# cyberfabric/cyberfabric-core

Measured on AMD Instinct MI355X. Metric: tokens/sec + p50 TTFT via llm-gateway REST /v1/chat/completions, higher is better.
Workload: dtype bf16; 1 GPU; model=llama3-8b, global_batch=2048, seq_len=512, parallelism=dp1(worker fleet)

## Files before the change

csrc/bindings.cpp:

```cpp
#include <torch/extension.h>

#include <c10/hip/HIPStream.h>
#include <hip/hip_bf16.h>

#include <stdexcept>

using bf16 = __hip_bfloat16;

void launch_rmsnorm(bf16*, const bf16*, const bf16*, float, long, int,
                    hipStream_t);
void launch_fused_add_rmsnorm(bf16*, bf16*, const bf16*, float, long, int,
                              hipStream_t);
void launch_rope_kv_append(bf16*, bf16*, const bf16*, const long*,
                           const float*, const long*, bf16*, bf16*, long,
                           int, int, int, int, long, long, long, bool,
                           hipStream_t);
void launch_paged_attn(bf16*, const bf16*, const bf16*, const bf16*,
                       const int*, const int*, const int*, long, int, int,
                       int, int, int, float, long, float*, int, bool,
                       hipStream_t);
void launch_attn_prefill_mfma(bf16*, const bf16*, const bf16*,
                              const bf16*, const int*, int, int, int, int,
                              int, float, long, long, long, hipStream_t);
void launch_attn_prefill_paged_mfma(bf16*, const bf16*, const bf16*,
                                    const bf16*, const int*, const int*,
                                    const int*, int, int, int, int, int, int,
                                    int, float, long, bool, hipStream_t);
void launch_silu_mul(bf16*, const bf16*, long, int, hipStream_t);
void launch_quant_fp8(unsigned char*, float*, const bf16*, long, int, long,
                      hipStream_t);
void launch_fused_add_rmsnorm_fp8(unsigned char*, float*, const bf16*,
                                  bf16*, const bf16*, float, long, int,
                                  hipStream_t);
void launch_silu_mul_fp8(unsigned char*, float*, const bf16*, long, int,
                         hipStream_t);
void launch_moe_align(int*, int*, int*, const int*, int, int, int,
                      hipStream_t);
void launch_moe_gemm(bf16*, float*, const bf16*, const bf16*, const int*,
                     const int*, int, int, int, int, int, hipStream_t);
void launch_moe_combine(bf16*, const bf16*, const float*, const int*, long,
                        int, int, hipStream_t);
void launch_moe_gemm_fp8(bf16*, float*, const unsigned char*, const float*,
                         const unsigned char*, const float*, const int*,
                         const int*, int, int, int, int, int, hipStream_t);
void launch_greedy_sample(long*, const bf16*, long, int, hipStream_t);
void launch_inv_cdf_sample(long*, const float*, const float*, long, int,
                           hipStream_t);

namespace {

hipStream_t stream() {
  return c10::hip::getCurrentHIPStream().stream();
}

void check(const torch::Tensor& t, torch::ScalarType dt, const char* name) {
  TORCH_CHECK(t.is_cuda(), name, " must be on GPU");
  TORCH_CHECK(t.is_contiguous(), name, " must be contiguous");
  TORCH_CHECK(t.scalar_type() == dt, name, " has wrong dtype");
}

bf16* bf(torch::Tensor& t) { return reinterpret_cast<bf16*>(t.data_ptr()); }
const bf16* cbf(const torch::Tensor& t) {
  return reinterpret_cast<const bf16*>(t.data_ptr());
}

void rmsnorm(torch::Tensor out, torch::Tensor x, torch::Tensor w,
             double eps) {
  check(out, torch::kBFloat16, "out");
  check(x, torch::kBFloat16, "x");
  check(w, torch::kBFloat16, "w");
  const int hidden = (int)x.size(-1);
  TORCH_CHECK(hidden % 8 == 0 && hidden <= 16384, "hidden size");
  launch_rmsnorm(bf(out), cbf(x), cbf(w), (float)eps, x.numel() / hidden,
                 hidden, stream());
}

void fused_add_rmsnorm(torch::Tensor x, torch::Tensor residual,
                       torch::Tensor w, double eps) {
  check(x, torch::kBFloat16, "x");
  check(residual, torch::kBFloat16, "residual");
// ... 132 lines not shown
  launch_attn_prefill_paged_mfma(
      bf(out), cbf(q), cbf(k_cache), cbf(v_cache),
      block_tables.data_ptr<int>(), seq_start.data_ptr<int>(),
      ctx_start.data_ptr<int>(), S, (int)max_seqlen, H, KV,
      (int)q.size(2), (int)block_tables.size(1), (int)k_cache.size(2),
      (float)scale, q.stride(0), kv_fp8, stream());
}

void silu_mul(torch::Tensor out, torch::Tensor x) {
  check(out, torch::kBFloat16, "out");
  check(x, torch::kBFloat16, "x");
  const int inter = (int)out.size(-1);
  TORCH_CHECK(x.size(-1) == 2 * inter && inter % 8 == 0, "shape");
  launch_silu_mul(bf(out), cbf(x), out.numel() / inter, inter, stream());
}

void greedy_sample(torch::Tensor out, torch::Tensor logits) {
  check(out, torch::kInt64, "out");
  check(logits, torch::kBFloat16, "logits");
  launch_greedy_sample(out.data_ptr<long>(), cbf(logits), logits.size(0),
                       (int)logits.size(1), stream());
}

void inv_cdf_sample(torch::Tensor out, torch::Tensor logits,
                    torch::Tensor uniform) {
  check(out, torch::kInt64, "out");
  check(logits, torch::kFloat32, "logits");
  check(uniform, torch::kFloat32, "uniform");
  launch_inv_cdf_sample(out.data_ptr<long>(), logits.data_ptr<float>(),
                        uniform.data_ptr<float>(), logits.size(0),
                        (int)logits.size(1), stream());
}

}


unsigned char* u8(torch::Tensor& t) {
  return reinterpret_cast<unsigned char*>(t.data_ptr());
}

void quant_fp8(torch::Tensor out, torch::Tensor scales, torch::Tensor x) {
  check(out, torch::kFloat8_e4m3fn, "out");
  check(scales, torch::kFloat, "scales");
  TORCH_CHECK(x.is_cuda() && x.scalar_type() == torch::kBFloat16, "x");
  const int hidden = (int)x.size(-1);
  TORCH_CHECK(x.stride(-1) == 1, "x inner dim must be contiguous");
  const long rows = x.numel() / hidden;
  const long stride = x.dim() > 1 ? x.stride(0) : hidden;
  launch_quant_fp8(u8(out), scales.data_ptr<float>(), cbf(x), rows, hidden,
                   stride, stream());
}

void fused_add_rmsnorm_fp8(torch::Tensor out, torch::Tensor scales,
                           torch::Tensor x, torch::Tensor residual,
                           torch::Tensor w, double eps) {
  check(out, torch::kFloat8_e4m3fn, "out");
  check(scales, torch::kFloat, "scales");
  check(x, torch::kBFloat16, "x");
  check(residual, torch::kBFloat16, "residual");
  check(w, torch::kBFloat16, "w");
  const int hidden = (int)x.size(-1);
  launch_fused_add_rmsnorm_fp8(u8(out), scales.data_ptr<float>(), cbf(x),
                               bf(residual), cbf(w), (float)eps,
                               x.numel() / hidden, hidden, stream());
}

// ... 76 lines not shown
    TORCH_CHECK(skw.has_value(),
                "moe_gemm_fp8: splitk>1 needs a workspace");
    check(*skw, torch::kFloat, "skw");
    TORCH_CHECK(skw->numel() >= splitk * out.numel(),
                "moe_gemm_fp8: workspace too small");
    skp = skw->data_ptr<float>();
  }
  launch_moe_gemm_fp8(bf(out), skp, u8(xq), xs.data_ptr<float>(), u8(wq),
                      ws.data_ptr<float>(), sorted_ids.data_ptr<int>(),
                      tile_expert.data_ptr<int>(),
                      (int)tile_expert.numel(), (int)wq.size(1),
                      (int)wq.size(2), (int)gather_div, (int)splitk,
                      stream());
}

PYBIND11_MODULE(TORCH_EXTENSION_NAME, m) {
  m.doc() = "HyperSpot-AMD gfx950 (CDNA4) kernels";
  m.def("rmsnorm", &rmsnorm);
  m.def("quant_fp8", &quant_fp8);
  m.def("fused_add_rmsnorm_fp8", &fused_add_rmsnorm_fp8);
  m.def("silu_mul_fp8", &silu_mul_fp8);
  m.def("moe_align", &moe_align);
  m.def("moe_gemm", &moe_gemm);
  m.def("moe_combine", &moe_combine);
  m.def("moe_gemm_fp8", &moe_gemm_fp8);
  m.def("fused_add_rmsnorm", &fused_add_rmsnorm);
  m.def("rope_kv_append", &rope_kv_append);
  m.def("paged_attn", &paged_attn);
  m.def("attn_prefill_mfma", &attn_prefill_mfma);
  m.def("attn_prefill_paged_mfma", &attn_prefill_paged_mfma);
  m.def("silu_mul", &silu_mul);
  m.def("greedy_sample", &greedy_sample);
  m.def("inv_cdf_sample", &inv_cdf_sample);
}
```

hyperspot/engine/config.py:

```python

from __future__ import annotations

from dataclasses import dataclass, field
from typing import Optional


@dataclass
class ModelSpec:

    name: str
    hidden_size: int
    num_layers: int
    num_heads: int
    num_kv_heads: int
    head_dim: int
    intermediate_size: int
    vocab_size: int
    rope_theta: float = 500000.0
    rms_eps: float = 1e-5
    max_position: int = 8192
    tie_embeddings: bool = False
    num_experts: int = 0
    num_experts_per_tok: int = 0
    dtype: str = "bfloat16"
# ... 46 lines not shown
        name="tiny-moe", hidden_size=256, num_layers=2, num_heads=4,
        num_kv_heads=2, head_dim=64, intermediate_size=256, vocab_size=512,
        rope_theta=10000.0, max_position=1024, num_experts=4,
        num_experts_per_tok=2,
    ),
}


def get_model_spec(name: str) -> ModelSpec:
    key = name.lower()
    if key not in _PRESETS:
        raise KeyError(f"unknown model preset '{name}' (have: {sorted(_PRESETS)})")
    return _PRESETS[key]


@dataclass
class EngineConfig:

    model: str = "llama3-8b"
    block_size: int = 16
    max_num_seqs: int = 256
    max_num_batched_tokens: int = 8192
    max_model_len: int = 8192
    gpu_memory_utilization: float = 0.90
    num_gpu_blocks: Optional[int] = None
    enforce_eager: bool = False
    tp_size: int = 1
    ep_size: int = 1
    dtype: str = "bfloat16"
    quant: Optional[str] = None
    kv_dtype: str = "bfloat16"
    enable_prefix_caching: bool = False
    prefill_paged_mfma: bool = False
    seed: int = 0
    graph_batch_sizes: tuple = (1, 2, 4, 8, 16, 24, 32, 48, 64, 96, 128,
                                192, 256, 384, 512, 768, 1024, 1536, 2048)
    prefill_graph_sizes: tuple = (128, 256, 512, 1024, 2048)

    def spec(self) -> ModelSpec:
        return get_model_spec(self.model)


@dataclass
class SamplingParams:

    temperature: float = 1.0
    top_p: float = 1.0
    top_k: int = 0
    max_tokens: int = 128
    min_tokens: int = 0
    stop_token_ids: tuple = ()
    ignore_eos: bool = False
    seed: Optional[int] = None
    response_format: Optional[str] = None
    response_schema: Optional[dict] = None
    tool_names: tuple = ()

    @property
    def greedy(self) -> bool:
        return self.temperature == 0.0
```

hyperspot/engine/engine.py:

```python

from __future__ import annotations

import itertools
import logging
import time
from typing import List, Optional

from .config import EngineConfig, SamplingParams
from .model_runner import ModelRunner
from .request import FinishReason, Request, StepOutput
from .scheduler import Scheduler

log = logging.getLogger(__name__)


class LLMEngine:
    def __init__(self, config: EngineConfig, device: Optional[str] = None,
                 eos_token_id: Optional[int] = None):
        t0 = time.monotonic()
        self.config = config
        self.runner = ModelRunner(config, device=device)
        self.scheduler = Scheduler(config, self.runner.block_manager)
        self.eos_token_id = eos_token_id
        self._id_counter = itertools.count()
        log.info("engine up: model=%s blocks=%d device=%s (%.1fs)",
                 config.model, self.runner.num_blocks, self.runner.device,
                 time.monotonic() - t0)

    def add_request(self, prompt_token_ids: List[int],
                    sampling: Optional[SamplingParams] = None,
                    request_id: Optional[str] = None,
                    tenant_id: str = "default") -> str:
        rid = request_id or f"req-{next(self._id_counter)}"
        req = Request(request_id=rid,
                      prompt_token_ids=list(prompt_token_ids),
                      sampling=sampling or SamplingParams(),
                      tenant_id=tenant_id)
        self.scheduler.add(req)
        return rid

    def abort_request(self, request_id: str) -> None:
        self.scheduler.abort(request_id)

    def has_work(self) -> bool:
        return self.scheduler.has_work()

    @property
    def num_running(self) -> int:
        return len(self.scheduler.running)

    @property
    def num_waiting(self) -> int:
        return len(self.scheduler.waiting)

    def step(self) -> List[StepOutput]:
        batch = self.scheduler.schedule()
        if batch.empty:
            return []
        tokens = self.runner.execute(batch)
        outputs: List[StepOutput] = []
        bm = self.runner.block_manager
        for req, tok in zip(batch.requests, tokens.tolist()):
            if batch.mode == "prefill" and bm.enable_prefix_caching:
                bm.commit_hashes(req.request_id, req.num_computed_tokens)
            if batch.mode == "prefill" and \
                    req.num_computed_tokens < req.num_prompt_tokens:
                continue
            req.append_output(int(tok), self.eos_token_id)
            outputs.append(StepOutput(req.request_id, int(tok), req.finished,
                                      req.finish_reason))
        self.scheduler.finish_step()
        return outputs

    def capture_graphs(self) -> None:
        self.runner.capture_all_graphs()

    def embed(self, prompts):
        return self.runner.embed(prompts)

    def swap_weights(self, checkpoint_path: str) -> float:
        return self.runner.swap_weights(checkpoint_path)

    def save_checkpoint(self, path: str) -> None:
        from .checkpoint import save_checkpoint
        save_checkpoint(self.runner.model, path,
                        {"model": self.config.model})

    def generate(self, prompts: List[List[int]],
                 sampling: Optional[SamplingParams] = None):
        ids = [self.add_request(p, sampling) for p in prompts]
        results = {i: [] for i in ids}
        while self.has_work():
            for out in self.step():
                if out.request_id in results:
                    results[out.request_id].append(out.token_id)
        return [results[i] for i in ids]
```

hyperspot/engine/model_runner.py:

```python

from __future__ import annotations

import logging
from typing import Dict, List, Optional

import torch

from hyperspot import ops
from hyperspot.models import build_model
from hyperspot.models.llama import ForwardMeta

from .config import EngineConfig
from .kv_cache import (BlockManager, allocate_kv_caches,
                       compute_num_gpu_blocks)
from .request import Request
from .scheduler import ScheduledBatch

log = logging.getLogger(__name__)

_TUNABLEOP_LOADED = False


def _load_tunableop_results() -> None:
    global _TUNABLEOP_LOADED
    if _TUNABLEOP_LOADED:
        return
    _TUNABLEOP_LOADED = True
    import os
    path = os.path.join(os.path.dirname(os.path.dirname(
        os.path.dirname(os.path.abspath(__file__)))),
        "profiles", "tunableop_gfx950.csv")
    if not os.path.exists(path):
        return
    try:
        t = torch.cuda.tunable
        t.enable(True)
        t.tuning_enable(False)
        t.record_untuned_enable(False)
        t.read_file(path)
        log.info("TunableOp: loaded %s", path)
    except Exception as e:
        log.warning("TunableOp load failed: %s", e)


class ModelRunner:
    def __init__(self, config: EngineConfig, device: Optional[str] = None):
        self.config = config
        self.spec = config.spec()
        if config.max_model_len > self.spec.max_position:
            log.warning("max_model_len %d clamped to the model's "
                        "max_position %d", config.max_model_len,
                        self.spec.max_position)
            config.max_model_len = self.spec.max_position
        self.device = torch.device(
            device if device is not None
            else ("cuda" if torch.cuda.is_available() else "cpu"))
        self.dtype = torch.bfloat16 if self.device.type == "cuda" \
            else torch.float32
        torch.manual_seed(config.seed)
        if self.device.type == "cuda":
            _load_tunableop_results()
        from hyperspot.parallel.layers import set_init_device, set_quant_mode
        set_init_device(self.device)
        set_quant_mode(config.quant)
        self.model = build_model(self.spec, dtype=self.dtype).to(self.device)
        self.model.eval()
        self.num_blocks = compute_num_gpu_blocks(self.spec, config, self.device)
        kv_heads_local = self.spec.num_kv_heads // max(config.tp_size, 1)
        assert config.kv_dtype in ("bfloat16", "fp8"), config.kv_dtype
        kv_dt = torch.float8_e4m3fn if config.kv_dtype == "fp8"             else self.dtype
        self.kv_caches = allocate_kv_caches(
            self.spec.num_layers, self.num_blocks, kv_heads_local,
            config.block_size, self.spec.head_dim, kv_dt, self.device)
        self.max_blocks_per_seq = (config.max_model_len + config.block_size - 1) \
            // config.block_size
        self.block_manager = BlockManager(
            self.num_blocks, config.block_size,
            capacity=max(config.max_num_seqs * 2, 64),
            max_blocks_per_seq=self.max_blocks_per_seq,
            enable_prefix_caching=config.enable_prefix_caching)
        self._gen = torch.Generator().manual_seed(config.seed)
        pin = self.device.type == "cuda"
        cap = self.block_manager.capacity
        self._st_ids = torch.empty(cap, dtype=torch.long, pin_memory=pin)
        self._st_pos = torch.empty(cap, dtype=torch.long, pin_memory=pin)
        self._st_slots = torch.empty(cap, dtype=torch.long, pin_memory=pin)
        self._st_lens = torch.empty(cap, dtype=torch.int32, pin_memory=pin)
        self._st_bt_flat = torch.empty(cap * self.max_blocks_per_seq,
                                       dtype=torch.int32, pin_memory=pin)
        self._guided_mask_cache: Dict[tuple, torch.Tensor] = {}
        self._graphs: Dict[int, torch.cuda.CUDAGraph] = {}
        self._graph_io: Dict[int, dict] = {}
        self._pgraphs: Dict[int, torch.cuda.CUDAGraph] = {}
        self._pgraph_io: Dict[int, dict] = {}
        self._graph_pool = None


    def _prefill_inputs(self, batch: ScheduledBatch):
        ids: List[int] = []
        pos: List[int] = []
        slots: List[int] = []
        starts = [0]
        logit_rows = []
        import numpy as np
        row_seq: List[int] = []
        tables = []
        bm = self.block_manager
        bs = bm.block_size
        fresh = True
        ctx_start: List[int] = []
        for si, req in enumerate(batch.requests):
            cs = req.chunk_start
            n = req.chunk_len or req.num_prompt_tokens
            ctx_start.append(cs)
            if cs > 0:
                fresh = False
            ids.extend(req.prompt_token_ids[cs:cs + n])
            pos.extend(range(cs, cs + n))
            row = bm.row_of[req.request_id]
            p = np.arange(cs, cs + n)
            s = bm.tables_np[row, p // bs].astype(np.int64) * bs + p % bs
            slots.extend(s.tolist())
            starts.append(starts[-1] + n)
            logit_rows.append(starts[-1] - 1)
            row_seq.extend([si] * n)
            tables.append(bm.table(req.request_id))
        max_t = max(len(t) for t in tables)
        bt = torch.zeros(len(tables), max_t, dtype=torch.int32)
# ... 108 lines not shown
            "input_ids": torch.zeros(T, dtype=torch.long, device=d),
            "positions": torch.zeros(T, dtype=torch.long, device=d),
            "slot_mapping": torch.full((T,), -1, dtype=torch.long,
                                       device=d),
            "lidx": torch.zeros(1, dtype=torch.long, device=d),
        }
        meta = ForwardMeta(
            mode="prefill", positions=io["positions"],
            slot_mapping=io["slot_mapping"],
            seq_start=torch.tensor([0, T], dtype=torch.int32, device=d),
            max_seqlen=T, fresh_prefill=True,
            logits_indices=io["lidx"])
        for _ in range(2):
            self.model(io["input_ids"], meta, self.kv_caches)
        torch.cuda.synchronize()
        g = torch.cuda.CUDAGraph()
        with torch.cuda.graph(g, pool=self._graph_pool):
            io["logits"] = self.model(io["input_ids"], meta,
                                      self.kv_caches)
        if self._graph_pool is None:
            self._graph_pool = g.pool()
        self._pgraphs[T] = g
        self._pgraph_io[T] = io

    def _decode_forward(self, input_ids, meta):
        B = input_ids.shape[0]
        bucket = self._bucket_for(B)
        if bucket is None or self.device.type != "cuda" \
                or self.config.enforce_eager:
            return self.model(input_ids, meta, self.kv_caches)
        if bucket not in self._graphs:
            self._capture(bucket)
        io = self._graph_io[bucket]
        io["input_ids"][:B] = input_ids
        io["input_ids"][B:] = 0
        io["positions"][:B] = meta.positions
        io["positions"][B:] = 0
        io["slot_mapping"][:B] = meta.slot_mapping
        io["slot_mapping"][B:] = -1
        io["block_tables"].zero_()
        io["block_tables"][:B, :meta.block_tables.shape[1]] = meta.block_tables
        io["seq_lens"][:B] = meta.seq_lens
        io["seq_lens"][B:] = 1
        self._graphs[bucket].replay()
        return io["logits"][:B]

    def _bucket_for(self, b: int) -> Optional[int]:
        for s in self.config.graph_batch_sizes:
            if s >= b:
                return s
        return None

    def _capture(self, bucket: int) -> None:
        d = self.device
        log.info("capturing decode hipGraph for batch=%d", bucket)
        io = {
            "input_ids": torch.zeros(bucket, dtype=torch.long, device=d),
            "positions": torch.zeros(bucket, dtype=torch.long, device=d),
            "slot_mapping": torch.full((bucket,), -1, dtype=torch.long, device=d),
            "block_tables": torch.zeros(bucket, self.max_blocks_per_seq,
                                        dtype=torch.int32, device=d),
            "seq_lens": torch.ones(bucket, dtype=torch.int32, device=d),
        }
        meta = ForwardMeta(mode="decode", positions=io["positions"],
                           slot_mapping=io["slot_mapping"],
                           block_tables=io["block_tables"],
                           seq_lens=io["seq_lens"])
        for _ in range(2):
            self.model(io["input_ids"], meta, self.kv_caches)
        torch.cuda.synchronize()
        g = torch.cuda.CUDAGraph()
        with torch.cuda.graph(g, pool=self._graph_pool):
            io["logits"] = self.model(io["input_ids"], meta, self.kv_caches)
        if self._graph_pool is None:
            self._graph_pool = g.pool()
        self._graphs[bucket] = g
        self._graph_io[bucket] = io

    @torch.inference_mode()
    def capture_all_graphs(self) -> None:
        if self.device.type != "cuda" or self.config.enforce_eager:
            return
        for b in self.config.graph_batch_sizes:
            if b <= self.config.max_num_seqs and b not in self._graphs:
                self._capture(b)
        for t in self.config.prefill_graph_sizes:
            if (t <= self.config.max_num_batched_tokens
                    and t <= self.config.max_model_len
                    and t not in self._pgraphs):
                self._capture_prefill(t)


    @torch.inference_mode()
    def embed(self, prompts: List[List[int]]) -> torch.Tensor:
        from .request import Request
        from .config import SamplingParams
        bm = self.block_manager
        fake = []
        try:
            for i, p in enumerate(prompts):
                rid = f"__embed_{i}"
                bm.allocate(rid, len(p))
                fake.append(Request(request_id=rid, prompt_token_ids=list(p),
                                    sampling=SamplingParams()))
            batch = ScheduledBatch(mode="prefill", requests=fake,
                                   num_tokens=sum(len(p) for p in prompts))
            input_ids, meta = self._prefill_inputs(batch)
            meta.return_hidden = True
            hidden = self.model(input_ids, meta, self.kv_caches).float()
            out = torch.empty(len(prompts), hidden.shape[-1],
                              dtype=torch.float32, device=hidden.device)
            ss = meta.seq_start
            for i in range(len(prompts)):
                out[i] = hidden[int(ss[i]):int(ss[i + 1])].mean(0)
        finally:
            for i in range(len(prompts)):
                bm.free(f"__embed_{i}")
        return out.cpu()

    def swap_weights(self, checkpoint_path: str) -> float:
        from .checkpoint import load_checkpoint_into
        return load_checkpoint_into(self.model, checkpoint_path)

# ... 77 lines not shown
```

hyperspot/engine/scheduler.py:

```python

from __future__ import annotations

from collections import deque
from dataclasses import dataclass, field
from typing import Deque, List, Optional

from .config import EngineConfig
from .kv_cache import BlockManager
from .request import Request, RequestState


@dataclass
class ScheduledBatch:
    mode: str
    requests: List[Request] = field(default_factory=list)
    num_tokens: int = 0

    @property
    def empty(self) -> bool:
        return not self.requests


class Scheduler:
    def __init__(self, config: EngineConfig, block_manager: BlockManager):
        self.config = config
        self.bm = block_manager
        self.waiting: Deque[Request] = deque()
        self.running: List[Request] = []
        self.watermark = max(1, int(0.01 * block_manager.num_blocks))

    def add(self, req: Request) -> None:
        self.waiting.append(req)

    def abort(self, request_id: str) -> None:
        for q in (self.waiting, self.running):
            for r in list(q):
                if r.request_id == request_id:
                    q.remove(r)
                    if r.request_id in self.bm.row_of:
                        self.bm.free(r.request_id)
                    r.state = RequestState.FINISHED

    def has_work(self) -> bool:
        return bool(self.waiting or self.running)

    def schedule(self) -> ScheduledBatch:
        batch = self._schedule_prefill()
        if not batch.empty:
            return batch
        return self._schedule_decode()

    def _schedule_prefill(self) -> ScheduledBatch:
        batch = ScheduledBatch(mode="prefill")
        budget = self.config.max_num_batched_tokens
        completed = []
        while self.waiting and budget > 0:
            req = self.waiting[0]
            total = req.num_prompt_tokens
            if total > self.config.max_model_len:
                self.waiting.popleft()
                req.state = RequestState.FINISHED
                continue
            done = req.num_computed_tokens
            if done == 0 and len(self.running) + len(batch.requests)                     >= self.config.max_num_seqs:
                break
            if done == 0 and self.bm.enable_prefix_caching:
                if not self.bm.can_allocate(total, self.watermark):
                    break
                cached = self.bm.allocate_with_prefix(
                    req.request_id, total, req.prompt_token_ids)
                req.num_computed_tokens = done = cached
                req.blocks_preallocated = True
            chunk = min(total - done, budget)
            if chunk <= 0:
                break
            if getattr(req, "blocks_preallocated", False):
                pass
            elif done == 0:
                if not self.bm.can_allocate(chunk, self.watermark):
                    break
                self.bm.allocate(req.request_id, chunk)
            else:
                if not self.bm.can_extend(req.request_id, chunk,
                                          self.watermark):
                    break
                self.bm.extend(req.request_id, chunk)
            req.chunk_start, req.chunk_len = done, chunk
            req.num_computed_tokens = done + chunk
            batch.requests.append(req)
            budget -= chunk
            batch.num_tokens += chunk
            if req.num_computed_tokens == total:
                self.waiting.popleft()
                req.state = RequestState.RUNNING
                completed.append(req)
        self.running.extend(completed)
        return batch

    def _schedule_decode(self) -> ScheduledBatch:
        batch = ScheduledBatch(mode="decode")
        while self.running:
            need = sum(1 for req in self.running
                       if self.bm.tokens_of(req.request_id)
                       % self.bm.block_size == 0)
            if need <= self.bm.num_free:
                break
            victim = self.running.pop()
            self.bm.free(victim.request_id)
            victim.state = RequestState.PREEMPTED
            victim.prompt_token_ids = victim.prompt_token_ids + victim.output_token_ids
            victim.output_token_ids = []
            victim.num_computed_tokens = 0
            victim.blocks_preallocated = False
            self.waiting.appendleft(victim)
        batch.requests = list(self.running)
        batch.num_tokens = len(batch.requests)
        return batch

    def finish_step(self) -> List[Request]:
        done = [r for r in self.running if r.finished]
        for r in done:
            self.bm.free(r.request_id)
        self.running = [r for r in self.running if not r.finished]
        return done
```

hyperspot/ops/__init__.py:

```python

from __future__ import annotations

from typing import NamedTuple

import torch

from . import torch_ref

_C = None
_C_ERR: Exception | None = None
try:
    from hyperspot import _C as _C
except Exception as e:
    _C_ERR = e


def have_native() -> bool:
    return _C is not None


def _native():
    if _C is None:
        raise RuntimeError(
            "hyperspot._C (gfx950 HIP extension) is not built but a GPU tensor "
# ... 197 lines not shown

def moe_ffn_fp8(xq: "QTensor", w13q: torch.Tensor, w13s: torch.Tensor,
                w2q: torch.Tensor, w2s: torch.Tensor,
                weights: torch.Tensor, ids: torch.Tensor) -> torch.Tensor:
    T, H = xq.data.shape
    K = ids.shape[1]
    E = w13q.shape[0]
    TK = T * K
    ntiles = (TK + E * (MOE_BM - 1) + MOE_BM - 1) // MOE_BM
    P = ntiles * MOE_BM
    dev = xq.data.device
    flat = ids.reshape(-1).to(torch.int32)
    sorted_ids = torch.empty(P, dtype=torch.int32, device=dev)
    tile_expert = torch.empty(ntiles, dtype=torch.int32, device=dev)
    inv_pos = torch.empty(TK, dtype=torch.int32, device=dev)
    n = _native()
    n.moe_align(sorted_ids, tile_expert, inv_pos, flat, E)
    I2 = w13q.shape[1]
    h1 = torch.empty(P, I2, dtype=torch.bfloat16, device=dev)
    s1, ws1 = _moe_splitk(ntiles * (I2 // 128), H // 128, P * I2, dev)
    n.moe_gemm_fp8(h1, xq.data, xq.scale, w13q, w13s, sorted_ids,
                   tile_expert, K, s1, ws1)
    a = silu_mul_q(h1)
    y = torch.empty(P, H, dtype=torch.bfloat16, device=dev)
    I = w2q.shape[2]
    s2, ws2 = _moe_splitk(ntiles * (H // 128), I // 128, P * H, dev)
    n.moe_gemm_fp8(y, a.data, a.scale, w2q, w2s, sorted_ids, tile_expert,
                   0, s2, ws2)
    out = torch.empty(T, H, dtype=torch.bfloat16, device=dev)
    n.moe_combine(out, y, weights.float().contiguous(), inv_pos, K)
    return out


def greedy_sample(logits: torch.Tensor) -> torch.Tensor:
    if logits.is_cuda:
        out = torch.empty(logits.shape[0], dtype=torch.long,
                          device=logits.device)
        _native().greedy_sample(out, logits)
        return out
    return logits.float().argmax(-1)


def sample(logits: torch.Tensor, temperature: torch.Tensor,
           top_p: torch.Tensor, top_k: torch.Tensor,
           uniform: torch.Tensor) -> torch.Tensor:
    if not logits.is_cuda:
        return torch_ref.sample(logits, temperature, top_p, top_k, uniform)
    if bool((temperature == 0).all()):
        return greedy_sample(logits)
    lf = logits.float()
    B, V = lf.shape
    t = temperature.clamp_min(1e-6)[:, None]
    row = lf / t
    if bool((top_k > 0).any()):
        k = top_k.clamp(0, V)
        kth = torch.where(
            k > 0,
            row.topk(int(k.max().clamp(min=1)), dim=-1).values.gather(
                1, (k.clamp(min=1) - 1)[:, None]).squeeze(1),
            torch.full_like(row[:, 0], float("-inf")))
        row = torch.where(row < kth[:, None], float("-inf"), row)
    if bool((top_p < 1.0).any()):
        sp, idx = row.softmax(-1).sort(descending=True)
        cum = sp.cumsum(-1)
        drop = (cum - sp) >= top_p[:, None]
        row = row.masked_fill(drop.gather(1, idx.argsort(-1)), float("-inf"))
    out = torch.empty(B, dtype=torch.long, device=logits.device)
    _native().inv_cdf_sample(out, row, uniform)
    greedy = temperature == 0
    if bool(greedy.any()):
        out = torch.where(greedy, greedy_sample(logits), out)
    return out
```

hyperspot/ops/torch_ref.py:

```python

from __future__ import annotations

import torch


def rmsnorm(x: torch.Tensor, weight: torch.Tensor, eps: float) -> torch.Tensor:
    dt = x.dtype
    xf = x.float()
    out = xf * torch.rsqrt(xf.pow(2).mean(-1, keepdim=True) + eps)
    return (out * weight.float()).to(dt)


def fused_add_rmsnorm(x: torch.Tensor, residual: torch.Tensor,
                      weight: torch.Tensor, eps: float):
    res = (residual.float() + x.float())
    out = res * torch.rsqrt(res.pow(2).mean(-1, keepdim=True) + eps)
    out = (out * weight.float()).to(x.dtype)
    return out, res.to(x.dtype)


def rope_cos_sin(positions: torch.Tensor, head_dim: int, theta: float,
                 dtype: torch.dtype = torch.float32) -> torch.Tensor:
    inv = 1.0 / (theta ** (torch.arange(0, head_dim, 2, dtype=torch.float32,
                                        device=positions.device) / head_dim))
# ... 69 lines not shown
        p = att.softmax(-1)
        o = torch.einsum("kgn,knd->kgd", p, v)
        out[t] = o.reshape(H, D).to(q.dtype)
    return out


def prefill_attn(q: torch.Tensor, k: torch.Tensor, v: torch.Tensor,
                 seq_start: torch.Tensor, scale: float) -> torch.Tensor:
    T, H, D = q.shape
    KV = k.shape[1]
    group = H // KV
    out = torch.empty_like(q)
    for i in range(seq_start.numel() - 1):
        s, e = int(seq_start[i]), int(seq_start[i + 1])
        n = e - s
        qs = q[s:e].float().view(n, KV, group, D)
        ks = k[s:e].float()
        vs = v[s:e].float()
        att = torch.einsum("mkgd,nkd->kgmn", qs, ks) * scale
        mask = torch.full((n, n), float("-inf"), device=q.device).triu(1)
        att = att + mask
        p = att.softmax(-1)
        o = torch.einsum("kgmn,nkd->mkgd", p, vs)
        out[s:e] = o.reshape(n, H, D).to(q.dtype)
    return out


def silu_mul(gate_up: torch.Tensor) -> torch.Tensor:
    i = gate_up.shape[-1] // 2
    g, u = gate_up[..., :i].float(), gate_up[..., i:].float()
    return (torch.nn.functional.silu(g) * u).to(gate_up.dtype)


def sample(logits: torch.Tensor, temperature: torch.Tensor,
           top_p: torch.Tensor, top_k: torch.Tensor,
           uniform: torch.Tensor) -> torch.Tensor:
    B, V = logits.shape
    out = torch.empty(B, dtype=torch.long, device=logits.device)
    lf = logits.float()
    for b in range(B):
        t = float(temperature[b])
        if t == 0.0:
            out[b] = int(lf[b].argmax())
            continue
        row = lf[b] / t
        k = int(top_k[b])
        if 0 < k < V:
            kth = row.topk(k).values[-1]
            row = row.masked_fill(row < kth, float("-inf"))
        probs = row.softmax(-1)
        p = float(top_p[b])
        if p < 1.0:
            sp, idx = probs.sort(descending=True)
            cum = sp.cumsum(-1)
            keep = cum - sp < p
            sp = sp * keep
            sp = sp / sp.sum()
            c = sp.cumsum(-1)
            j = int(torch.searchsorted(c, uniform[b].to(c.dtype), right=False).clamp(max=V - 1))
            out[b] = int(idx[j])
        else:
            c = probs.cumsum(-1)
            j = int(torch.searchsorted(c, uniform[b].to(c.dtype), right=False).clamp(max=V - 1))
            out[b] = j
    return out

# ... 8 lines not shown
```

hyperspot/serving/worker.py:

```python

from __future__ import annotations

import argparse
import json
import logging
import os
import queue
import socket
import threading
import time

log = logging.getLogger("hyperspot.worker")


class WorkerState:

    def __init__(self, engine, tokenizer, tp: int = 1):
        self.engine = engine
        self.tokenizer = tokenizer
        self.tp = tp
        self.lock = threading.Lock()
        self.new_work = threading.Condition(self.lock)
        self.streams = {}
        self.started = {}
# ... 21 lines not shown

    def submit(self, rid, prompt_ids, sampling):
        q = queue.Queue()
        with self.new_work:
            self.streams[rid] = q
            self.started[rid] = len(prompt_ids)
            self.engine.add_request(prompt_ids, sampling, request_id=rid)
            if self.tp > 1:
                self.pending_ops.append(
                    ("add", rid, prompt_ids, sampling.__dict__.copy()))
            self.new_work.notify()
        return q

    def abort(self, rid):
        with self.submit_mu:
            self.pending_submits = [t for t in self.pending_submits
                                    if t[0] != rid]
        with self.new_work:
            self.engine.abort_request(rid)
            q = self.streams.pop(rid, None)
            self.started.pop(rid, None)
            mux = self.mux_of.pop(rid, None)
            if mux is not None:
                mux.forget(rid)
            if q is not None:
                q.put(None)
            if self.tp > 1:
                self.pending_ops.append(("abort", rid))
                self.new_work.notify()

    def exec_collective(self, kind, arg, timeout=900):
        if self.tp == 1:
            with self.lock:
                return self._exec(kind, arg)
        q = queue.Queue()
        with self.new_work:
            self.pending_exec.append((kind, arg, q))
            self.new_work.notify()
        res = q.get(timeout=timeout)
        if isinstance(res, Exception):
            raise res
        return res

    def drain_mux_inputs(self):
        for mux in list(self.mux_channels):
            data_parts = []
            dead = False
            while True:
                try:
                    chunk = mux.sock.recv(1 << 20, socket.MSG_DONTWAIT)
                except (BlockingIOError, InterruptedError):
                    break
                except OSError:
                    dead = True
                    break
                if not chunk:
                    dead = True
                    break
                data_parts.append(chunk)
            if data_parts:
                mux.rx_buf += b"".join(data_parts)
                while True:
                    nl = mux.rx_buf.find(b"\n")
                    if nl < 0:
                        break
                    line = mux.rx_buf[:nl]
                    mux.rx_buf = mux.rx_buf[nl + 1:]
# ... 64 lines not shown

    def _exec(self, kind, arg):
        if kind == "swap":
            return self.engine.swap_weights(arg)
        if kind == "save":
            return self.engine.save_checkpoint(arg)
        if kind == "embed":
            return self.engine.embed(arg)
        raise ValueError(kind)

    def step_loop(self):
        try:
            self._step_loop()
        except Exception:
            log.exception("stepping thread crashed; exiting worker for "
                          "watchdog respawn")
            os._exit(17)

    def _step_loop(self):
        import torch.distributed as dist
        while not self.stop:
            if self.bench_req is not None:
                self._run_bench()
                continue
            self.drain_mux_inputs()
            with self.new_work:
                while not self.engine.has_work() and not self.stop                         and not self.pending_ops and self.bench_req is None                         and not self.pending_exec and not self.pending_submits:
                    self.new_work.wait(timeout=0.5)
                    if self.mux_channels:
                        break
                if self.stop:
                    if self.tp > 1:
                        dist.broadcast_object_list([("stop",)], src=0)
                    return
                if self.bench_req is not None:
                    continue
                while self.pending_exec:
                    kind, arg, q = self.pending_exec.pop(0)
                    dist.broadcast_object_list([("exec", kind, arg)],
                                               src=0)
                    try:
                        q.put(self._exec(kind, arg))
                    except Exception as e:
                        q.put(e)
                self._drain_submits_locked()
                if not self.engine.has_work() and not self.pending_ops:
                    continue
                if self.hold_decode and (self._ramp_incomplete()
                                         or self._only_decode_left()):
                    self.new_work.wait(timeout=0.02)
                    continue
                if self.tp > 1:
                    ops = self.pending_ops
                    self.pending_ops = []
                    dist.broadcast_object_list([("step", ops)], src=0)
                outputs = self.engine.step()
            self._fanout(outputs)

    def _fanout(self, outputs):
        per_mux = None
        for out in outputs:
            rid = out.request_id
            mux = self.mux_of.get(rid)
            if mux is not None:
                if per_mux is None:
                    per_mux = {}
                fr = ((out.finish_reason.value if out.finish_reason
                       else "stop") if out.finished else None)
                per_mux.setdefault(mux, []).append(
                    (rid, out.token_id, fr))
                if out.finished:
                    self.mux_of.pop(rid, None)
                continue
            q = self.streams.get(rid)
            if q is not None:
                q.put(out)
                if out.finished:
                    self.streams.pop(rid, None)
                    self.started.pop(rid, None)
        if per_mux:
            for mux, raw in per_mux.items():
                mux.send_outputs(raw)

    def _one_step(self):
        import torch.distributed as dist
        self.drain_mux_inputs()
        t0 = time.perf_counter()
        with self.new_work:
            t1 = time.perf_counter()
            self._drain_submits_locked()
            if self.tp > 1:
                ops = self.pending_ops
                self.pending_ops = []
                dist.broadcast_object_list([("step", ops)], src=0)
            outputs = self.engine.step()
        t2 = time.perf_counter()
        self._fanout(outputs)
        t3 = time.perf_counter()
        self._bt_lock += t1 - t0
        self._bt_step += t2 - t1
        self._bt_fanout += t3 - t2
        self._last_outputs = outputs
        return len(outputs)

    def _sync(self):
        import torch
        import torch.distributed as dist
        if self.tp > 1:
            dist.broadcast_object_list([("bench_sync",)], src=0)
        if torch.cuda.is_available():
            torch.cuda.synchronize()
        if self.tp > 1:
            dist.barrier()

    def _run_bench(self):
        warmup, steps, start_at, want_tokens = self.bench_req
        self.bench_req = None
        self.hold_decode = False
        try:
            while time.time() < start_at:
                time.sleep(0.001)
            for _ in range(warmup):
                self._one_step()
            self._sync()
            self._bt_lock = self._bt_step = self._bt_fanout = 0.0
            t0 = time.time()
            produced = 0
            for _ in range(steps):
                produced += self._one_step()
            self._sync()
            t1 = time.time()
            extra = {}
            if want_tokens:
                extra["last_tokens"] = [o.token_id
                                        for o in self._last_outputs]
            self.bench_result.put({
                **extra,
                "event": "bench_done", "t0": t0, "t1": t1,
                "elapsed": t1 - t0, "produced": produced,
                "steps": steps, "warmup": warmup,
                "ms_lock": self._bt_lock / steps * 1000,
                "ms_engine": self._bt_step / steps * 1000,
                "ms_fanout": self._bt_fanout / steps * 1000})
        except Exception as e:
            self.bench_result.put({"event": "error",
                                   "message": f"bench failed: {e}"})


class MuxChannel:

    MAX_PENDING = 4096

    def __init__(self, sock: socket.socket):
        self.sock = sock
        self.rx_buf = b""
        self.rx_event = threading.Event()
        self.rids = set()
        self.pending = []
        self.cv = threading.Condition()
        self.dead = False
        self.meta = {}
        self.meta_add = []
# ... 454 lines not shown
```

Before: 34810 tokens/s.

## Pipeline greedy decode steps with on-device state advance inside graphs

Adds a decode_advance GPU kernel that derives the next step's input ids, positions, seq_lens, slot mapping and block-table updates from the previously sampled tokens and a small pinned control buffer. Greedy sampling is captured into the decode graph. The engine gains a step_pipelined path that launches step N+1 before collecting step N's tokens, so host scheduling and output fanout overlap GPU work. The cost is much more complex bookkeeping: deferred frees, abort handling, a ring of pinned buffers, and drains before any non-greedy or scheduling change, all of which risk correctness bugs.

```diff
diff --git a/csrc/bindings.cpp b/csrc/bindings.cpp
--- a/csrc/bindings.cpp
+++ b/csrc/bindings.cpp
@@ -46,6 +46,8 @@
 void launch_greedy_sample(long*, const bf16*, long, int, hipStream_t);
 void launch_inv_cdf_sample(long*, const float*, const float*, long, int,
                            hipStream_t);
+void launch_decode_advance(long*, long*, int*, long*, int*, const long*,
+                           const int*, int, int, int, hipStream_t);
 
 namespace {
 
@@ -244,6 +246,35 @@
                         (int)logits.size(1), stream());
 }
 
+void decode_advance(torch::Tensor input_ids, torch::Tensor positions,
+                    torch::Tensor seq_lens, torch::Tensor slot_mapping,
+                    torch::Tensor block_tables, torch::Tensor sampled_prev,
+                    torch::Tensor ctl, int64_t page) {
+  check(input_ids, torch::kInt64, "input_ids");
+  check(positions, torch::kInt64, "positions");
+  check(seq_lens, torch::kInt32, "seq_lens");
+  check(slot_mapping, torch::kInt64, "slot_mapping");
+  check(block_tables, torch::kInt32, "block_tables");
+  check(sampled_prev, torch::kInt64, "sampled_prev");
+  check(ctl, torch::kInt32, "ctl");
+  const int64_t rows = input_ids.numel();
+  TORCH_CHECK(rows > 0 && page > 0, "empty decode_advance");
+  TORCH_CHECK(block_tables.dim() == 2 && block_tables.size(0) == rows,
+              "block_tables must be [rows, max_blocks]");
+  TORCH_CHECK(positions.numel() == rows && seq_lens.numel() == rows &&
+                  slot_mapping.numel() == rows &&
+                  sampled_prev.numel() == rows,
+              "per-row tensors must have `rows` elements");
+  TORCH_CHECK(ctl.numel() >= 4 * rows + 1, "ctl must hold 4*rows+1 ints");
+  launch_decode_advance(input_ids.data_ptr<long>(), positions.data_ptr<long>(),
+                        seq_lens.data_ptr<int>(),
+                        slot_mapping.data_ptr<long>(),
+                        block_tables.data_ptr<int>(),
+                        sampled_prev.data_ptr<long>(), ctl.data_ptr<int>(),
+                        (int)rows, (int)block_tables.size(1), (int)page,
+                        stream());
+}
+
 }
 
 
@@ -386,4 +417,5 @@
   m.def("silu_mul", &silu_mul);
   m.def("greedy_sample", &greedy_sample);
   m.def("inv_cdf_sample", &inv_cdf_sample);
-}
+  m.def("decode_advance", &decode_advance);
+}
diff --git a/csrc/decode_state.hip b/csrc/decode_state.hip
--- /dev/null
+++ b/csrc/decode_state.hip
@@ -0,0 +1,56 @@
+
+#include <hip/hip_runtime.h>
+
+__global__ __launch_bounds__(256) void decode_advance_kernel(
+    long* __restrict__ input_ids, long* __restrict__ positions,
+    int* __restrict__ seq_lens, long* __restrict__ slot_mapping,
+    int* __restrict__ block_tables, const long* __restrict__ sampled_prev,
+    const int* __restrict__ ctl, int rows, int max_blocks, int page) {
+  const int r = blockIdx.x * 256 + threadIdx.x;
+  if (r >= rows) return;
+  const int n_live = ctl[4 * rows];
+  if (n_live < 0) return;
+  const int src = ctl[r];
+  if (r >= n_live || src < -1 || src >= rows) {
+    input_ids[r] = 0;
+    positions[r] = 0;
+    seq_lens[r] = 1;
+    slot_mapping[r] = -1;
+    return;
+  }
+  long pos;
+  if (src >= 0) {
+    input_ids[r] = sampled_prev[src];
+    pos = positions[r] + 1;
+  } else {
+    input_ids[r] = (long)ctl[2 * rows + r];
+    pos = (long)ctl[3 * rows + r];
+  }
+  positions[r] = pos;
+  seq_lens[r] = (int)pos + 1;
+  const long bi = pos / page;
+  if (pos < 0 || bi >= max_blocks) {
+    slot_mapping[r] = -1;
+    return;
+  }
+  int* trow = block_tables + (long)r * max_blocks;
+  const int nb = ctl[rows + r];
+  int blk;
+  if (nb >= 0) {
+    trow[bi] = nb;
+    blk = nb;
+  } else {
+    blk = trow[bi];
+  }
+  slot_mapping[r] = (long)blk * page + pos % page;
+}
+
+void launch_decode_advance(long* input_ids, long* positions, int* seq_lens,
+                           long* slot_mapping, int* block_tables,
+                           const long* sampled_prev, const int* ctl, int rows,
+                           int max_blocks, int page, hipStream_t stream) {
+  decode_advance_kernel<<<dim3((unsigned)((rows + 255) / 256)), 256, 0,
+                          stream>>>(input_ids, positions, seq_lens,
+                                    slot_mapping, block_tables, sampled_prev,
+                                    ctl, rows, max_blocks, page);
+}
diff --git a/hyperspot/engine/config.py b/hyperspot/engine/config.py
--- a/hyperspot/engine/config.py
+++ b/hyperspot/engine/config.py
@@ -102,6 +102,7 @@
     kv_dtype: str = "bfloat16"
     enable_prefix_caching: bool = False
     prefill_paged_mfma: bool = False
+    pipeline_decode: bool = True
     seed: int = 0
     graph_batch_sizes: tuple = (1, 2, 4, 8, 16, 24, 32, 48, 64, 96, 128,
                                 192, 256, 384, 512, 768, 1024, 1536, 2048)
diff --git a/hyperspot/engine/engine.py b/hyperspot/engine/engine.py
--- a/hyperspot/engine/engine.py
+++ b/hyperspot/engine/engine.py
@@ -23,6 +23,7 @@
         self.scheduler = Scheduler(config, self.runner.block_manager)
         self.eos_token_id = eos_token_id
         self._id_counter = itertools.count()
+        self._inflight = None
         log.info("engine up: model=%s blocks=%d device=%s (%.1fs)",
                  config.model, self.runner.num_blocks, self.runner.device,
                  time.monotonic() - t0)
@@ -40,10 +41,16 @@
         return rid
 
     def abort_request(self, request_id: str) -> None:
-        self.scheduler.abort(request_id)
+        h = self._inflight
+        if h is not None and h.runs(request_id):
+            self.scheduler.abort(request_id, free=False)
+            h.deferred_free.append(request_id)
+        else:
+            self.scheduler.abort(request_id)
+        self.runner.pipe_drop(request_id)
 
     def has_work(self) -> bool:
-        return self.scheduler.has_work()
+        return self.scheduler.has_work() or self._inflight is not None
 
     @property
     def num_running(self) -> int:
@@ -54,11 +61,12 @@
         return len(self.scheduler.waiting)
 
     def step(self) -> List[StepOutput]:
+        outputs: List[StepOutput] = self.drain()
         batch = self.scheduler.schedule()
         if batch.empty:
-            return []
+            return outputs
         tokens = self.runner.execute(batch)
-        outputs: List[StepOutput] = []
+        self.runner.pipe_invalidate()
         bm = self.runner.block_manager
         for req, tok in zip(batch.requests, tokens.tolist()):
             if batch.mode == "prefill" and bm.enable_prefix_caching:
@@ -70,6 +78,67 @@
             outputs.append(StepOutput(req.request_id, int(tok), req.finished,
                                       req.finish_reason))
         self.scheduler.finish_step()
+        return outputs
+
+
+    def _pipe_eligible(self) -> bool:
+        for r in self.scheduler.running:
+            sp = r.sampling
+            if sp.temperature != 0 or sp.response_schema is not None \
+                    or sp.response_format in ("json", "tool_call"):
+                return False
+        return True
+
+    def step_pipelined(self) -> List[StepOutput]:
+        cfg = self.config
+        sch = self.scheduler
+        rn = self.runner
+        fast = (cfg.pipeline_decode and cfg.tp_size == 1
+                and not sch.waiting and bool(sch.running))
+        seed = None
+        if fast and (not rn.pipe_valid() or rn.pipe_stale()):
+            if self._inflight is not None:
+                return self.drain()
+            fast = self._pipe_eligible()
+            seed = sch.running
+        if fast:
+            h = rn.pipe_launch(seed)
+            if h is not None:
+                prev, self._inflight = self._inflight, h
+                return self._collect(prev) if prev is not None else []
+        if self._inflight is not None:
+            return self.drain()
+        return self.step()
+
+    def drain(self) -> List[StepOutput]:
+        h, self._inflight = self._inflight, None
+        return self._collect(h) if h is not None else []
+
+    def _collect(self, h) -> List[StepOutput]:
+        outputs: List[StepOutput] = []
+        done = []
+        eos = self.eos_token_id
+        for req, tok in self.runner.pipe_collect(h):
+            if req.finished:
+                continue
+            req.append_output(tok, eos)
+            outputs.append(StepOutput(req.request_id, tok, req.finished,
+                                      req.finish_reason))
+            if req.finished:
+                done.append(req)
+        bm = self.runner.block_manager
+        if done:
+            nxt = self._inflight
+            for r in done:
+                self.runner.pipe_drop(r.request_id)
+                if nxt is not None and nxt.runs(r.request_id):
+                    nxt.deferred_free.append(r.request_id)
+                else:
+                    bm.free(r.request_id)
+            self.scheduler.running = [r for r in self.scheduler.running
+                                      if not r.finished]
+        for rid in h.deferred_free:
+            bm.free(rid)
         return outputs
 
     def capture_graphs(self) -> None:
diff --git a/hyperspot/engine/model_runner.py b/hyperspot/engine/model_runner.py
--- a/hyperspot/engine/model_runner.py
+++ b/hyperspot/engine/model_runner.py
@@ -41,6 +41,23 @@
         log.info("TunableOp: loaded %s", path)
     except Exception as e:
         log.warning("TunableOp load failed: %s", e)
+
+
+class PipeStep:
+
+    __slots__ = ("reqs", "slots", "ring", "deferred_free", "_rids")
+
+    def __init__(self, reqs, slots, ring):
+        self.reqs = reqs
+        self.slots = slots
+        self.ring = ring
+        self.deferred_free: List[str] = []
+        self._rids = None
+
+    def runs(self, request_id: str) -> bool:
+        if self._rids is None:
+            self._rids = {r.request_id for r in self.reqs}
+        return request_id in self._rids
 
 
 class ModelRunner:
@@ -94,6 +111,15 @@
         self._pgraphs: Dict[int, torch.cuda.CUDAGraph] = {}
         self._pgraph_io: Dict[int, dict] = {}
         self._graph_pool = None
+        self._pipe: Optional[dict] = None
+        self._pipe_eager_io: Optional[dict] = None
+        self._pipe_seq = 0
+        self._pipe_ring = [
+            {"ctl": torch.empty(4 * cap + 4, dtype=torch.int32,
+                                pin_memory=pin),
+             "tok": torch.empty(cap, dtype=torch.long, pin_memory=pin),
+             "event": torch.cuda.Event() if pin else None}
+            for _ in range(4)]
 
 
     def _prefill_inputs(self, batch: ScheduledBatch):
@@ -268,6 +294,9 @@
         if bucket not in self._graphs:
             self._capture(bucket)
         io = self._graph_io[bucket]
+        if not io["passthrough"]:
+            io["ctl"][4 * bucket:].fill_(-1)
+            io["passthrough"] = True
         io["input_ids"][:B] = input_ids
         io["input_ids"][B:] = 0
         io["positions"][:B] = meta.positions
@@ -297,17 +326,26 @@
             "block_tables": torch.zeros(bucket, self.max_blocks_per_seq,
                                         dtype=torch.int32, device=d),
             "seq_lens": torch.ones(bucket, dtype=torch.int32, device=d),
+            "sampled": torch.zeros(bucket, dtype=torch.long, device=d),
+            "ctl": torch.full((4 * bucket + 4,), -1, dtype=torch.int32,
+                              device=d),
+            "passthrough": True,
         }
         meta = ForwardMeta(mode="decode", positions=io["positions"],
                            slot_mapping=io["slot_mapping"],
                            block_tables=io["block_tables"],
                            seq_lens=io["seq_lens"])
         for _ in range(2):
-            self.model(io["input_ids"], meta, self.kv_caches)
+            self._pipe_head(io)
+            ops.greedy_sample(
+                self.model(io["input_ids"], meta, self.kv_caches),
+                out=io["sampled"])
         torch.cuda.synchronize()
         g = torch.cuda.CUDAGraph()
         with torch.cuda.graph(g, pool=self._graph_pool):
+            self._pipe_head(io)
             io["logits"] = self.model(io["input_ids"], meta, self.kv_caches)
+            ops.greedy_sample(io["logits"], out=io["sampled"])
         if self._graph_pool is None:
             self._graph_pool = g.pool()
         self._graphs[bucket] = g
@@ -325,6 +363,153 @@
                     and t <= self.config.max_model_len
                     and t not in self._pgraphs):
                 self._capture_prefill(t)
+
+
+    def _pipe_head(self, io: dict) -> None:
+        ops.decode_advance(io["input_ids"], io["positions"], io["seq_lens"],
+                           io["slot_mapping"], io["block_tables"],
+                           io["sampled"], io["ctl"], self.config.block_size)
+
+    def pipe_invalidate(self) -> None:
+        self._pipe = None
+
+    def pipe_valid(self) -> bool:
+        return self._pipe is not None
+
+    def pipe_drop(self, request_id: str) -> None:
+        p = self._pipe
+        if p is not None:
+            s = p["slot_of"].get(request_id)
+            if s is not None:
+                p["alive"][s] = False
+
+    def pipe_stale(self) -> bool:
+        p = self._pipe
+        if p is None:
+            return False
+        n = int(p["alive"].sum())
+        if n == 0:
+            return False
+        if p["graph"]:
+            return self._bucket_for(n) != p["bucket"]
+        return n * 2 <= len(p["reqs"])
+
+    def _pipe_seed(self, reqs: List[Request]) -> None:
+        import numpy as np
+        bm = self.block_manager
+        B = len(reqs)
+        bucket = self._bucket_for(B)
+        graph = (bucket is not None and self.device.type == "cuda"
+                 and not self.config.enforce_eager)
+        if graph:
+            if bucket not in self._graphs:
+                self._capture(bucket)
+            io = self._graph_io[bucket]
+            nrows = bucket
+        else:
+            full = self._pipe_eager_io
+            if full is None:
+                cap, d = bm.capacity, self.device
+                full = self._pipe_eager_io = {
+                    "input_ids": torch.zeros(cap, dtype=torch.long, device=d),
+                    "positions": torch.zeros(cap, dtype=torch.long, device=d),
+                    "slot_mapping": torch.full((cap,), -1, dtype=torch.long,
+                                               device=d),
+                    "block_tables": torch.zeros(cap, self.max_blocks_per_seq,
+                                                dtype=torch.int32, device=d),
+                    "seq_lens": torch.ones(cap, dtype=torch.int32, device=d),
+                    "sampled": torch.zeros(cap, dtype=torch.long, device=d),
+                    "ctl": torch.full((4 * cap + 4,), -1, dtype=torch.int32,
+                                      device=d),
+                }
+            nrows = B
+            io = {k: v[:nrows] for k, v in full.items() if k != "ctl"}
+            io["ctl"] = full["ctl"][:4 * nrows + 4]
+        self._pipe = {
+            "graph": graph, "bucket": bucket, "io": io, "nrows": nrows,
+            "reqs": list(reqs), "fresh": True,
+            "slot_of": {r.request_id: i for i, r in enumerate(reqs)},
+            "rows": np.fromiter((bm.row_of[r.request_id] for r in reqs),
+                                dtype=np.int64, count=B),
+            "alive": np.ones(B, dtype=bool),
+            "remaining": np.fromiter(
+                (r.sampling.max_tokens - r.num_generated for r in reqs),
+                dtype=np.int64, count=B),
+        }
+
+    @torch.inference_mode()
+    def pipe_launch(self, seed_reqs: Optional[List[Request]] = None):
+        import numpy as np
+        bm = self.block_manager
+        bs = bm.block_size
+        if seed_reqs is not None:
+            self._pipe_seed(seed_reqs)
+        p = self._pipe
+        idx = np.nonzero(p["alive"] & (p["remaining"] > 0))[0]
+        if idx.size == 0:
+            return None
+        rows = p["rows"][idx]
+        n = bm.tokens_np[rows].copy()
+        boundary = n % bs == 0
+        if int(boundary.sum()) > bm.num_free:
+            if p["fresh"]:
+                self._pipe = None
+            return None
+        bm.append_slots_batch(rows)
+        R = p["nrows"]
+        io = p["io"]
+        ring = self._pipe_ring[self._pipe_seq % len(self._pipe_ring)]
+        self._pipe_seq += 1
+        ctl = ring["ctl"].numpy()[:4 * R + 4]
+        c = ctl[:4 * R].reshape(4, R)
+        c[0].fill(-2)
+        c[1].fill(-1)
+        d = self.device
+        nb = d.type == "cuda"
+        if p["fresh"]:
+            reqs = p["reqs"]
+            c[0][idx] = -1
+            c[2][idx] = np.fromiter((reqs[i].last_token_id for i in idx),
+                                    dtype=np.int64, count=idx.size)
+            c[3][idx] = n
+            max_nt = int(bm.ntables_np[rows].max())
+            bt_stage = self._st_bt_flat[:idx.size * max_nt].view(
+                idx.size, max_nt)
+            bt_stage.numpy()[:] = bm.tables_np[
+                rows[:, None], np.arange(max_nt)[None, :]]
+            io["block_tables"][:idx.size, :max_nt] = \
+                bt_stage.to(d, non_blocking=nb)
+            p["fresh"] = False
+        else:
+            c[0][idx] = idx
+            c[1][idx[boundary]] = bm.tables_np[rows[boundary],
+                                               n[boundary] // bs]
+        ctl[4 * R] = int(idx[-1]) + 1
+        io["ctl"].copy_(ring["ctl"][:4 * R + 4], non_blocking=nb)
+        if p["graph"]:
+            io["passthrough"] = False
+            self._graphs[p["bucket"]].replay()
+        else:
+            self._pipe_head(io)
+            meta = ForwardMeta(mode="decode", positions=io["positions"],
+                               slot_mapping=io["slot_mapping"],
+                               block_tables=io["block_tables"],
+                               seq_lens=io["seq_lens"])
+            ops.greedy_sample(
+                self.model(io["input_ids"], meta, self.kv_caches),
+                out=io["sampled"])
+        ring["tok"][:R].copy_(io["sampled"], non_blocking=nb)
+        if nb:
+            ring["event"].record()
+        p["remaining"][idx] -= 1
+        return PipeStep([p["reqs"][i] for i in idx], idx, ring)
+
+    def pipe_collect(self, step: "PipeStep"):
+        ev = step.ring["event"]
+        if ev is not None:
+            ev.synchronize()
+        toks = step.ring["tok"].numpy()[step.slots].tolist()
+        return zip(step.reqs, toks)
 
 
     @torch.inference_mode()
diff --git a/hyperspot/engine/scheduler.py b/hyperspot/engine/scheduler.py
--- a/hyperspot/engine/scheduler.py
+++ b/hyperspot/engine/scheduler.py
@@ -32,12 +32,12 @@
     def add(self, req: Request) -> None:
         self.waiting.append(req)
 
-    def abort(self, request_id: str) -> None:
+    def abort(self, request_id: str, free: bool = True) -> None:
         for q in (self.waiting, self.running):
             for r in list(q):
                 if r.request_id == request_id:
                     q.remove(r)
-                    if r.request_id in self.bm.row_of:
+                    if free and r.request_id in self.bm.row_of:
                         self.bm.free(r.request_id)
                     r.state = RequestState.FINISHED
 
@@ -99,11 +99,14 @@
 
     def _schedule_decode(self) -> ScheduledBatch:
         batch = ScheduledBatch(mode="decode")
-        while self.running:
-            need = sum(1 for req in self.running
-                       if self.bm.tokens_of(req.request_id)
-                       % self.bm.block_size == 0)
-            if need <= self.bm.num_free:
+        import numpy as np
+        bm = self.bm
+        while self.running and len(self.running) > bm.num_free:
+            rows = np.fromiter((bm.row_of[r.request_id]
+                                for r in self.running), dtype=np.int64,
+                               count=len(self.running))
+            need = int((bm.tokens_np[rows] % bm.block_size == 0).sum())
+            if need <= bm.num_free:
                 break
             victim = self.running.pop()
             self.bm.free(victim.request_id)
@@ -119,6 +122,8 @@
 
     def finish_step(self) -> List[Request]:
         done = [r for r in self.running if r.finished]
+        if not done:
+            return done
         for r in done:
             self.bm.free(r.request_id)
         self.running = [r for r in self.running if not r.finished]
diff --git a/hyperspot/ops/__init__.py b/hyperspot/ops/__init__.py
--- a/hyperspot/ops/__init__.py
+++ b/hyperspot/ops/__init__.py
@@ -253,13 +253,31 @@
     return out
 
 
-def greedy_sample(logits: torch.Tensor) -> torch.Tensor:
+def greedy_sample(logits: torch.Tensor,
+                  out: torch.Tensor | None = None) -> torch.Tensor:
     if logits.is_cuda:
-        out = torch.empty(logits.shape[0], dtype=torch.long,
-                          device=logits.device)
+        if out is None:
+            out = torch.empty(logits.shape[0], dtype=torch.long,
+                              device=logits.device)
         _native().greedy_sample(out, logits)
         return out
-    return logits.float().argmax(-1)
+    res = logits.float().argmax(-1)
+    if out is not None:
+        out.copy_(res)
+        return out
+    return res
+
+
+def decode_advance(input_ids: torch.Tensor, positions: torch.Tensor,
+                   seq_lens: torch.Tensor, slot_mapping: torch.Tensor,
+                   block_tables: torch.Tensor, sampled_prev: torch.Tensor,
+                   ctl: torch.Tensor, page: int) -> None:
+    if input_ids.is_cuda:
+        _native().decode_advance(input_ids, positions, seq_lens, slot_mapping,
+                                 block_tables, sampled_prev, ctl, page)
+        return
+    torch_ref.decode_advance(input_ids, positions, seq_lens, slot_mapping,
+                             block_tables, sampled_prev, ctl, page)
 
 
 def sample(logits: torch.Tensor, temperature: torch.Tensor,
diff --git a/hyperspot/ops/torch_ref.py b/hyperspot/ops/torch_ref.py
--- a/hyperspot/ops/torch_ref.py
+++ b/hyperspot/ops/torch_ref.py
@@ -125,6 +125,35 @@
     return (torch.nn.functional.silu(g) * u).to(gate_up.dtype)
 
 
+def decode_advance(input_ids: torch.Tensor, positions: torch.Tensor,
+                   seq_lens: torch.Tensor, slot_mapping: torch.Tensor,
+                   block_tables: torch.Tensor, sampled_prev: torch.Tensor,
+                   ctl: torch.Tensor, page: int) -> None:
+    rows = input_ids.numel()
+    max_blocks = block_tables.shape[1]
+    n_live = int(ctl[4 * rows])
+    if n_live < 0:
+        return
+    c = ctl[:4 * rows].view(4, rows).long()
+    src, new_blk, host_ids, host_pos = c[0], c[1], c[2], c[3]
+    r = torch.arange(rows, device=input_ids.device)
+    live = (r < n_live) & (src >= -1) & (src < rows)
+    dev = live & (src >= 0)
+    ids = torch.where(dev, sampled_prev[src.clamp(0, rows - 1)], host_ids)
+    pos = torch.where(dev, positions + 1, host_pos)
+    input_ids.copy_(torch.where(live, ids, torch.zeros_like(ids)))
+    positions.copy_(torch.where(live, pos, torch.zeros_like(pos)))
+    seq_lens.copy_(torch.where(live, pos + 1,
+                               torch.ones_like(pos)).to(seq_lens.dtype))
+    bi = torch.div(pos, page, rounding_mode="floor")
+    ok = live & (pos >= 0) & (bi < max_blocks)
+    inst = ok & (new_blk >= 0)
+    block_tables[r[inst], bi[inst]] = new_blk[inst].to(block_tables.dtype)
+    blk = block_tables[r, bi.clamp(0, max_blocks - 1)].long()
+    slot_mapping.copy_(torch.where(ok, blk * page + pos % page,
+                                   torch.full_like(pos, -1)))
+
+
 def sample(logits: torch.Tensor, temperature: torch.Tensor,
            top_p: torch.Tensor, top_k: torch.Tensor,
            uniform: torch.Tensor) -> torch.Tensor:
diff --git a/hyperspot/serving/worker.py b/hyperspot/serving/worker.py
--- a/hyperspot/serving/worker.py
+++ b/hyperspot/serving/worker.py
@@ -77,7 +77,11 @@
     def exec_collective(self, kind, arg, timeout=900):
         if self.tp == 1:
             with self.lock:
-                return self._exec(kind, arg)
+                drained = self.engine.drain()
+                try:
+                    return self._exec(kind, arg)
+                finally:
+                    self._fanout(drained)
         q = queue.Queue()
         with self.new_work:
             self.pending_exec.append((kind, arg, q))
@@ -208,9 +212,12 @@
                 if self.stop:
                     if self.tp > 1:
                         dist.broadcast_object_list([("stop",)], src=0)
+                    self._fanout(self.engine.drain())
                     return
                 if self.bench_req is not None:
                     continue
+                if self.pending_exec:
+                    self._fanout(self.engine.drain())
                 while self.pending_exec:
                     kind, arg, q = self.pending_exec.pop(0)
                     dist.broadcast_object_list([("exec", kind, arg)],
@@ -224,14 +231,18 @@
                     continue
                 if self.hold_decode and (self._ramp_incomplete()
                                          or self._only_decode_left()):
+                    self._fanout(self.engine.drain())
                     self.new_work.wait(timeout=0.02)
                     continue
                 if self.tp > 1:
                     ops = self.pending_ops
                     self.pending_ops = []
                     dist.broadcast_object_list([("step", ops)], src=0)
-                outputs = self.engine.step()
+                outputs = self.engine.step_pipelined()
             self._fanout(outputs)
+        with self.new_work:
+            outputs = self.engine.drain()
+        self._fanout(outputs)
 
     def _fanout(self, outputs):
         per_mux = None
@@ -258,25 +269,29 @@
             for mux, raw in per_mux.items():
                 mux.send_outputs(raw)
 
-    def _one_step(self):
+    def _one_step(self, drain=False):
         import torch.distributed as dist
         self.drain_mux_inputs()
         t0 = time.perf_counter()
         with self.new_work:
             t1 = time.perf_counter()
             self._drain_submits_locked()
-            if self.tp > 1:
-                ops = self.pending_ops
-                self.pending_ops = []
-                dist.broadcast_object_list([("step", ops)], src=0)
-            outputs = self.engine.step()
+            if drain:
+                outputs = self.engine.drain()
+            else:
+                if self.tp > 1:
+                    ops = self.pending_ops
+                    self.pending_ops = []
+                    dist.broadcast_object_list([("step", ops)], src=0)
+                outputs = self.engine.step_pipelined()
         t2 = time.perf_counter()
         self._fanout(outputs)
         t3 = time.perf_counter()
         self._bt_lock += t1 - t0
         self._bt_step += t2 - t1
         self._bt_fanout += t3 - t2
-        self._last_outputs = outputs
+        if outputs or not drain:
+            self._last_outputs = outputs
         return len(outputs)
 
     def _sync(self):
@@ -299,11 +314,13 @@
             for _ in range(warmup):
                 self._one_step()
             self._sync()
+            self._one_step(drain=True)
             self._bt_lock = self._bt_step = self._bt_fanout = 0.0
             t0 = time.time()
             produced = 0
             for _ in range(steps):
                 produced += self._one_step()
+            produced += self._one_step(drain=True)
             self._sync()
             t1 = time.time()
             extra = {}
```

After: 39920 tokens/s, median of 6. 14.7% higher.
